# cropinghigh/sdrpp-dvbs-demodulator

Hardware: AMD Instinct MI355X
Metric: Msymbols/s demod+FEC, DVB-S2 8PSK 3/4 normal-frame @50 LDPC iters (higher is better)
Workload: dtype int8 (FEC) / f32 (demod); 1 GPU; DVB-S2 8PSK 3/4 normal FECFRAME (MODCOD 14), pilots off, 27.5 Msym/s-class streams at 2 sps, carrier offset 1e-3 rad/sample, clock error ~10 ppm, Es/N0 11 dB, 50 forced LDPC iterations, IQ in -> BBFRAMEs out; streams_per_gpu=4096, symbols_per_frame=21690, distinct_signal_blocks=64, parallelism=independent transponder streams sharded over GPUs, no data-path collective, fec_pipelined_across_steps=True, ranks_seen_by_backend=1, backend=none

## Files before the change

sdrpp-dvbs-demodulator_amd/csrc/bch_kernel.hip:

```cpp
#include <hip/hip_runtime.h>
#include <stdint.h>
#include "kernels.h"

namespace s2 {

struct GfDev {
    const uint16_t* __restrict__ LOG;
    const uint16_t* __restrict__ EXP;
    int N;
    __device__ __forceinline__ uint16_t imul(uint16_t a, uint16_t b) const {
        uint16_t tmp = (uint16_t)(a + b);
        return (N - (int)a <= (int)b) ? (uint16_t)(tmp - N) : tmp;
    }
    __device__ __forceinline__ uint16_t idiv(uint16_t a, uint16_t b) const {
        uint16_t tmp = (uint16_t)(a - b);
        return (a < b) ? (uint16_t)(tmp + N) : tmp;
    }
    __device__ __forceinline__ uint16_t vmul(uint16_t a, uint16_t b) const { return (!a || !b) ? (uint16_t)0 : EXP[imul(LOG[a], LOG[b])]; }
    __device__ __forceinline__ uint16_t vdiv(uint16_t a, uint16_t b) const { return !a ? (uint16_t)0 : EXP[idiv(LOG[a], LOG[b])]; }
    __device__ __forceinline__ uint16_t vmuli(uint16_t a, uint16_t idx) const { return !a ? (uint16_t)0 : EXP[imul(LOG[a], idx)]; }
};

__global__ __launch_bounds__(256) void bch_syndromes_kernel(BchDeviceCode C, const uint8_t* __restrict__ frames, int frame_stride,
                                                            int nbch, int nframes, uint16_t* __restrict__ syn_out, int32_t* __restrict__ todo,
                                                            int32_t* __restrict__ corrections) {
    __shared__ uint16_t tab[12 * 3 * 256];
    __shared__ uint16_t red[4][12];
    __shared__ uint16_t sfin[32];
    const int t = C.t;
    for (int i = threadIdx.x; i < t * 768; i += 256) tab[i] = C.d_syn_tab[i];
    __syncthreads();
    GfDev G{C.d_log, C.d_exp, C.N};
    const int nbytes = nbch / 8;
    const int chunk = (nbytes + 255) / 256;
    const int tid = threadIdx.x, lane = tid & 63, wave = tid >> 6;
    for (int f = blockIdx.x; f < nframes; f += gridDim.x) {
        const uint8_t* __restrict__ fr = frames + (size_t)f * frame_stride;
        int b0 = tid * chunk, b1 = min(b0 + chunk, nbytes);
        uint32_t P[12];
#pragma unroll
        for (int r = 0; r < 12; ++r) P[r] = 0;
        for (int b = b0; b < b1; ++b) {
            uint32_t byte = fr[b];
#pragma unroll
            for (int r = 0; r < 12; ++r)
                if (r < t) {
                    const uint16_t* T = tab + r * 768;
                    P[r] = (uint32_t)T[256 + (P[r] & 0xff)] ^ (uint32_t)T[512 + (P[r] >> 8)] ^ (uint32_t)T[byte];
                }
        }
        const long after = (b1 > b0) ? (long)nbch - 8L * b1 : 0;
#pragma unroll
        for (int r = 0; r < 12; ++r)
            if (r < t) {
                uint32_t v = P[r];
                if (v) {
                    int sh = (int)(((long)(2 * r + 1) * after) % C.N);
                    int e = (int)G.LOG[v] + sh;
                    if (e >= C.N) e -= C.N;
                    v = G.EXP[e];
                }
#pragma unroll
                for (int o = 32; o > 0; o >>= 1) v ^= __shfl_xor((int)v, o);
                if (lane == 0) red[wave][r] = (uint16_t)v;
            }
        __syncthreads();
        if (tid == 0) {
            for (int i = 0; i < 32; ++i) sfin[i] = 0;
            int nz = 0;
            for (int r = 0; r < t; ++r) { sfin[2 * r] = (uint16_t)(red[0][r] ^ red[1][r] ^ red[2][r] ^ red[3][r]); nz |= sfin[2 * r]; }
            if (nz)
                for (int k = 1; k <= t; ++k) sfin[2 * k - 1] = G.vmul(sfin[k - 1], sfin[k - 1]);
            sfin[31] = nz ? 1 : 0;
            if (nz) todo[2 + atomicAdd(&todo[0], 1)] = f;
            else if (corrections) corrections[f] = 0;
        }
        __syncthreads();
        if (tid < 32) syn_out[(size_t)f * 32 + tid] = sfin[tid];
        __syncthreads();
    }
}

__device__ __forceinline__ void xor_be_bit(uint8_t* buf, int pos) { buf[pos / 8] ^= (uint8_t)(1u << (7 - pos % 8)); }

constexpr int BCH_CT = 256;
constexpr int BCH_MAXDEG = 24;
__global__ __launch_bounds__(BCH_CT) void bch_correct_kernel(BchDeviceCode C, uint8_t* __restrict__ frames, int frame_stride, int nbch,
                                                             int kbch, int nframes, const uint16_t* __restrict__ syn_in, int32_t* __restrict__ todo,
                                                             int32_t* __restrict__ corrections) {
    __shared__ int s_item;
    __shared__ uint16_t s_loc[32];
    __shared__ uint16_t s_pos[32];
    __shared__ int s_deg, s_count, s_state;
    __shared__ uint16_t s_C[40], s_B[40], s_d;
    __shared__ uint16_t s_ev[32], s_mag[32];
    __shared__ int s_edeg;
    __shared__ uint16_t s_mul[BCH_MAXDEG][2][256];
    GfDev G{C.d_log, C.d_exp, C.N};
    const int NR = 2 * C.t;
    const int lane = threadIdx.x;
    const int ntodo = todo[0];
    while (true) {
        if (lane == 0) s_item = atomicAdd(&todo[1], 1);
        __syncthreads();
        const int item = s_item;
        __syncthreads();
        if (item >= ntodo) break;
        const int f = todo[2 + item];
        const uint16_t* __restrict__ syn = syn_in + (size_t)f * 32;
        if (lane <= NR) { s_C[lane] = lane == 0 ? 1 : 0; s_B[lane] = lane == 0 ? 1 : 0; }
        if (lane == 0) { s_state = 0; s_count = 0; s_deg = 0; }
        __syncthreads();
        int L = 0;
        for (int n = 0, m = 1; n < NR; ++n) {
            uint32_t prod = 0;
            if (lane >= 1 && lane <= L) prod = G.vmul(s_C[lane], syn[n - lane]);
            if (lane == 0) prod = syn[n];
#pragma unroll
            for (int o = 32; o > 0; o >>= 1) prod ^= (uint32_t)__shfl_xor((int)prod, o);
            if (lane == 0) s_d = (uint16_t)prod;
            __syncthreads();
            const uint16_t d = s_d;
            if (!d) {
                ++m;
            } else {
                uint16_t tnew = 0;
                if (lane <= NR) tnew = lane < m ? s_C[lane] : (uint16_t)(G.vmul(d, s_B[lane - m]) ^ s_C[lane]);
                const bool grow = 2 * L <= n;
                uint16_t bnew = 0;
                if (grow && lane <= NR) bnew = G.vdiv(s_C[lane], d);
                __syncthreads();
                if (lane <= NR) { s_C[lane] = tnew; if (grow) s_B[lane] = bnew; }
                if (grow) { L = n + 1 - L; m = 1; } else ++m;
            }
            __syncthreads();
        }
        if (lane == 0) {
            const uint16_t* Cc = s_C;
            int nonzero = 1;
            if (nonzero) {
                int deg = L;
                bool fail = false;
                while (!Cc[deg])
                    if (--deg < 0) { fail = true; break; }
                if (fail) {
                    s_state = -1;
                } else {
                    for (int i = 0; i <= NR; ++i) s_loc[i] = Cc[i];
                    s_deg = deg;
                    if (deg == 1) {
                        s_pos[0] = G.idiv(G.idiv(G.LOG[Cc[0]], G.LOG[Cc[1]]), 1);
                        s_count = 1; s_state = 2;
                    } else if (deg == 2) {
                        s_state = 2;
                        if (!Cc[1] || !Cc[0]) {
                            s_count = 0;
                        } else {
                            uint16_t a = Cc[2], b = Cc[1], c = Cc[0];
                            uint16_t ba = G.vdiv(b, a);
                            uint16_t Rr = C.d_imap[G.vdiv(G.vmul(a, c), G.vmul(b, b))];
                            if (!Rr) {
                                s_count = 0;
                            } else {
                                uint16_t v0 = G.vmul(ba, Rr);
                                s_pos[0] = G.idiv(G.LOG[v0], 1);
                                s_pos[1] = G.idiv(G.LOG[(uint16_t)(v0 ^ ba)], 1);
                                s_count = 2;
                            }
                        }
                    } else {
                        s_state = 1;
                    }
                }
            }
        }
        __syncthreads();
        if (s_state == 1) {
            const int deg = s_deg;
            for (int e = lane; e < deg * 512; e += BCH_CT) {
                const int j = e >> 9, h = (e >> 8) & 1, x = e & 255;
                const uint32_t v = h ? (uint32_t)x << 8 : (uint32_t)x;
                uint16_t r = 0;
                if (v && v <= (uint32_t)C.N) {
                    const int sh = (int)(((long)BCH_CT * (j + 1)) % C.N);
                    int lg2 = (int)G.LOG[v] + sh;
                    if (lg2 >= C.N) lg2 -= C.N;
                    r = G.EXP[lg2];
                }
                s_mul[j][h][x] = r;
            }
            uint32_t term[BCH_MAXDEG];
#pragma unroll
            for (int jj = 0; jj < BCH_MAXDEG; ++jj) {
                term[jj] = 0;
                if (jj < deg) {
                    const uint16_t c = s_loc[jj + 1];
                    if (c) {
                        const long e = (long)G.LOG[c] + (long)(jj + 1) * (long)(lane + 1);
                        term[jj] = G.EXP[(int)(e % C.N)];
                    }
                }
            }
            __syncthreads();
            const uint32_t c0 = s_loc[0];
            for (int i = lane; i < C.N; i += BCH_CT) {
                uint32_t sum = c0;
#pragma unroll
                for (int jj = 0; jj < BCH_MAXDEG; ++jj)
                    if (jj < deg) {
                        sum ^= term[jj];
                        term[jj] = (uint32_t)s_mul[jj][0][term[jj] & 255u] ^ (uint32_t)s_mul[jj][1][term[jj] >> 8];
                    }
                if (!sum) {
                    int slot = atomicAdd(&s_count, 1);
                    if (slot < 32) s_pos[slot] = (uint16_t)i;
                }
            }
            __syncthreads();
            if (lane == 0) s_state = 2;
        }
        __syncthreads();
        if (s_state == 2 && s_count >= s_deg && s_count <= 32 && s_count > 0) {
            const int count = s_count;
            const int etmp = count < NR - 1 ? count : NR - 1;
            if (lane <= etmp) {
                uint16_t e = G.vmul(syn[lane], s_loc[0]);
                for (int jj = 1; jj <= lane; ++jj) e ^= G.vmul(syn[lane - jj], s_loc[jj]);
                s_ev[lane] = e;
            }
            __syncthreads();
            if (lane == 0) {
                int edeg = -1;
                for (int i = 0; i <= etmp; ++i)
                    if (s_ev[i]) edeg = i;
                s_edeg = edeg;
            }
            __syncthreads();
            if (lane < count) {
                const int edeg = s_edeg;
                uint16_t root = G.imul(s_pos[lane], 1), tmp = root;
                uint16_t eval = s_ev[0];
                for (int jj = 1; jj <= edeg; ++jj) {
                    eval ^= G.vmuli(s_ev[jj], tmp);
                    tmp = G.imul(tmp, root);
                }
                uint16_t mag = 0;
                if (eval) {
                    uint16_t deriv = s_loc[1];
                    uint16_t root2 = G.imul(root, root), tmp2 = root2;
                    for (int jj = 3; jj <= count; jj += 2) {
                        deriv ^= G.vmuli(s_loc[jj], tmp2);
                        tmp2 = G.imul(tmp2, root2);
                    }
                    mag = G.EXP[G.idiv(G.LOG[eval], G.LOG[deriv])];
                }
                s_mag[lane] = mag;
            }
        }
        __syncthreads();
        if (lane == 0) {
            int result = 0;
            if (s_state == -1) {
                result = -1;
            } else if (s_state == 2) {
                const int deg = s_deg, count = s_count;
                if (count < deg || count > 32) {
                    result = -1;
                } else {
                    const uint16_t* magnitudes = s_mag;
                    const int short_by = C.K_full - kbch;
                    if (count <= 0) {
                        result = count;
                    } else {
                        bool bad = false;
                        for (int i = 0; i < count; ++i)
                            if ((int)s_pos[i] < short_by) bad = true;
                        if (!bad)
                            for (int i = 0; i < count; ++i)
                                if (1 < (int)magnitudes[i]) bad = true;
                        if (bad) {
                            result = -1;
                        } else {
                            uint8_t* fr = frames + (size_t)f * frame_stride;
                            for (int i = 0; i < count; ++i)
                                if (magnitudes[i]) { xor_be_bit(fr, (int)s_pos[i] - short_by); ++result; }
                        }
                    }
                }
            }
            if (corrections) corrections[f] = result;
        }
        __syncthreads();
    }
}

__global__ __launch_bounds__(256) void bb_descramble_kernel(const uint8_t* __restrict__ frames, int frame_stride,
                                                            const uint8_t* __restrict__ prbs, int out_bytes, int nframes,
                                                            uint8_t* __restrict__ out) {
    for (int f = blockIdx.y; f < nframes; f += gridDim.y)
        for (int b = blockIdx.x * 256 + threadIdx.x; b < out_bytes; b += gridDim.x * 256)
            out[(size_t)f * out_bytes + b] = frames[(size_t)f * frame_stride + b] ^ prbs[b];
}

hipError_t bch_syndromes_launch(const BchDeviceCode& C, const uint8_t* frames, int frame_stride, int nbch, int nframes,
                                uint16_t* syn, int32_t* todo, int32_t* corrections, hipStream_t stream) {
    hipError_t e = hipMemsetAsync(todo, 0, 2 * sizeof(int32_t), stream);
    if (e != hipSuccess) return e;
    int grid = nframes < 4096 ? nframes : 4096;
    hipLaunchKernelGGL(bch_syndromes_kernel, dim3(grid), dim3(256), 0, stream, C, frames, frame_stride, nbch, nframes, syn, todo, corrections);
    return hipGetLastError();
}
hipError_t bch_correct_launch(const BchDeviceCode& C, uint8_t* frames, int frame_stride, int nbch, int kbch, int nframes,
                              const uint16_t* syn, int32_t* todo, int32_t* corrections, hipStream_t stream) {
    int grid = nframes < 2048 ? nframes : 2048;
    hipLaunchKernelGGL(bch_correct_kernel, dim3(grid), dim3(BCH_CT), 0, stream, C, frames, frame_stride, nbch, kbch, nframes, syn, todo, corrections);
    return hipGetLastError();
}
hipError_t bb_descramble_launch(const uint8_t* frames, int frame_stride, const uint8_t* prbs, int out_bytes, int nframes,
                                uint8_t* out, hipStream_t stream) {
    int gx = (out_bytes + 255) / 256;
    if (gx > 32) gx = 32;
    int gy = nframes < 2048 ? nframes : 2048;
    hipLaunchKernelGGL(bb_descramble_kernel, dim3(gx, gy), dim3(256), 0, stream, frames, frame_stride, prbs, out_bytes, nframes, out);
    return hipGetLastError();
}

}
```

sdrpp-dvbs-demodulator_amd/csrc/capi.hip:

```cpp
#include "ctx.h"
#include <algorithm>
#include <climits>
#include <cstdlib>

using namespace s2;

namespace s2 {
std::atomic<long long> g_kernel_launches{0};
static thread_local std::string g_err;
std::string& last_error() { return g_err; }
int fail_hip(hipError_t e, const char* what) {
    g_err = std::string(what) + ": " + hipGetErrorString(e);
    return DVBS2GPU_ERR_HIP;
}
int dev_alloc(void** p, size_t bytes, bool zero, const char* what) {
    *p = nullptr;
    hipError_t e = hipMalloc(p, bytes);
    if (e == hipSuccess && zero) e = hipMemset(*p, 0, bytes);
    if (e == hipSuccess) return 0;
    dev_free(*p);
    *p = nullptr;
    return fail_hip(e, what);
}
void dev_free(void* p) { if (p) (void)hipFree(p); }
// ... 115 lines not shown
            if (!x || !y) return 0;
            int e = LOG[x] + LOG[y];
            if (e >= N) e -= N;
            return EXP[e];
        };
        for (int i = 2; i < N; i += 2) {
            uint16_t x = (uint16_t)i;
            uint16_t xxx = (uint16_t)(vmul(x, x) ^ x);
            if (xxx == (uint16_t)N) continue;
            IMAP[xxx] = x;
        }
        std::vector<uint16_t> tab((size_t)t * 768, 0);
        for (int r = 0; r < t; ++r) {
            int i = 2 * r + 1;
            uint16_t* T = &tab[(size_t)r * 768];
            for (int byte = 0; byte < 256; ++byte) {
                uint16_t v = 0;
                for (int b = 0; b < 8; ++b)
                    if ((byte >> (7 - b)) & 1) v ^= EXP[(int)(((long)i * (7 - b)) % N)];
                T[byte] = v;
            }
            uint16_t c = EXP[(int)(((long)i * 8) % N)];
            for (int x = 0; x < 256; ++x) {
                T[256 + x] = vmul((uint32_t)x, c);
                uint32_t hi = (uint32_t)x << 8;
                T[512 + x] = (hi < (uint32_t)Q) ? vmul(hi, c) : 0;
            }
        }
        BchCode D;
        D.m = m; D.t = t; D.N = N; D.K_full = N - m * t;
        int rc;
        if ((rc = upload(LOG, D.log, &D.d_log))) return rc;
        if ((rc = upload(EXP, D.exp, &D.d_exp))) return rc;
        if ((rc = upload(IMAP, D.imap, &D.d_imap))) return rc;
        if ((rc = upload(tab, D.syn_tab, &D.d_syn_tab))) return rc;
        it = ctx->bch.emplace(key, std::move(D)).first;
    }
    *out = &it->second;
    return 0;
}

// ... 3 lines not shown
    std::vector<uint8_t> seq(64800 / 8, 0);
    int sr = 0x4A80;
    for (int i = 0; i < 64800; i++) {
        int b = ((sr) ^ (sr >> 1)) & 1;
        seq[i / 8] |= (uint8_t)(b << (7 - (i % 8)));
        sr >>= 1;
        if (b) sr |= 0x4000;
    }
    return upload(seq, ctx->d_prbs);
}
}

namespace s2 {
static int ldpc_run(dvbs2gpu_ctx* ctx, const FecParams& f, const int8_t* d_llr, int nframes, int max_trials, int force,
                    uint8_t* d_hard, int hard_stride, int8_t* d_post, int32_t* d_trials, hipStream_t st, FecWs& W);
static int bch_run(dvbs2gpu_ctx* ctx, const FecParams& f, uint8_t* d_frames, int nframes, int32_t* d_corr, hipStream_t st, FecWs& W);

int fec_run(dvbs2gpu_ctx* ctx, const FecParams& f, const int8_t* d_llr, int nframes, int max_trials, int force, uint8_t* d_bbframes,
            int32_t* d_trials, int32_t* d_corr, hipStream_t st, FecWs* ws) {
    FecWs& W = ws ? *ws : ctx->fws;
    int rc;
    if ((rc = W.hard.ensure((size_t)nframes * (f.K / 8)))) return rc;
    uint8_t* hard = (uint8_t*)W.hard.p;
    {
        StageSpan sp(ctx->timers, ST_LDPC, st, nframes);
        if ((rc = ldpc_run(ctx, f, d_llr, nframes, max_trials, force, hard, f.K / 8, nullptr, d_trials, st, W))) return rc;
    }
    StageSpan sp(ctx->timers, ST_BCH, st, nframes);
    if ((rc = bch_run(ctx, f, hard, nframes, d_corr, st, W))) return rc;
    if ((rc = get_prbs(ctx))) return rc;
    HIP_TRY(bb_descramble_launch(hard, f.K / 8, ctx->d_prbs, f.kbch / 8, nframes, d_bbframes, st));
    return 0;
}
}

namespace s2 {
struct alignas(256) LdpcWorkCounter { unsigned int v[64]; };

enum class LdpcForm : int { lane = 0, wave = 1, split = 2 };
static LdpcForm ldpc_form(const dvbs2gpu_ctx* ctx, const LdpcDeviceCode& C) { return C.use_wave ? LdpcForm::wave : (C.use_split && ctx->ldpc_split) ? LdpcForm::split : LdpcForm::lane; }
struct LdpcGeometry { int grid, fpb; size_t rec_bytes; };
static LdpcGeometry ldpc_geometry(const dvbs2gpu_ctx* ctx, const LdpcDeviceCode& C, LdpcForm form, int nframes) {
    if (form == LdpcForm::wave) {
        const int per_cu = (int)((size_t)(160 * 1024 - LDPC_WAVE_LDS_RESERVE) / ldpc_wave_lds_bytes(C));
        return {std::min(ctx->num_cus * std::min(std::max(per_cu, 1), 16), nframes), 1, ldpc_wave_msg_bytes_per_frame(C)};
    }
    if (form == LdpcForm::split) return {std::min(ctx->num_cus * C.split_blocks_per_cu, nframes), 1, ldpc_split_msg_bytes_per_block(C)};
// ... 19 lines not shown
    }
    if (!d_hard) {
        if ((rc = W.hard.ensure((size_t)nframes * (f.K / 8)))) return rc;
        d_hard = (uint8_t*)W.hard.p; hard_stride = f.K / 8;
    }
    const LdpcJob J = {d_llr, nframes, max_trials, force, d_hard, hard_stride, d_post, d_trials, (uint32_t*)l_msg(W.msg.p), l_sgn(W.msg.p), l_counter(W.msg.p)->v,
                       G.grid, G.fpb, ctx->ldpc_split_fail_attempts, st};
    if (form == LdpcForm::wave) HIP_TRY(ldpc_wave_decode_launch(*C, J));
    else if (form == LdpcForm::lane) HIP_TRY(ldpc_decode_launch(*C, J));
    else if (nframes > 0) HIP_TRY(ldpc_split_decode_launch(*C, J));
    return 0;
}
}

namespace s2 {
static int bch_run(dvbs2gpu_ctx* ctx, const FecParams& f, uint8_t* d_frames, int nframes, int32_t* d_corr, hipStream_t st, FecWs& W) {
    BchDeviceCode* B;
    int rc = get_bch(ctx, f.bch_m, f.bch_t, &B);
    if (rc) return rc;
    ScratchLayout L;
    const auto l_syn = L.add<uint16_t>((size_t)nframes * 32); const auto l_todo = L.add<int32_t>((size_t)nframes + 2);
    if ((rc = W.syn.ensure(L.bytes()))) return rc;
    uint16_t* syn = l_syn(W.syn.p); int32_t* todo = l_todo(W.syn.p);
    HIP_TRY(bch_syndromes_launch(*B, d_frames, f.K / 8, f.K, nframes, syn, todo, d_corr, st));
    HIP_TRY(bch_correct_launch(*B, d_frames, f.K / 8, f.K, f.kbch, nframes, syn, todo, d_corr, st));
    return 0;
}
}

extern "C" {

const char* dvbs2gpu_version(void) { return "dvbs2gpu 0.1 (gfx950)"; }
int dvbs2gpu_preinit(void) {
    if (getenv("GPU_MAX_HW_QUEUES")) return 0;
    return setenv("GPU_MAX_HW_QUEUES", "12", 0) == 0 ? 1 : DVBS2GPU_ERR_ARG;
}
const char* dvbs2gpu_last_error(void) { return g_err.c_str(); }

int dvbs2gpu_device_count(void) {
    int n = 0;
// ... 259 lines not shown
    return rc ? rc : rc2;
}


int dvbs2gpu_bch_decode_batch(dvbs2gpu_ctx* ctx, int rate, int shortframes, uint8_t* d_frames, int nframes, int32_t* d_corrections,
                              void* stream) {
    if (!ctx || nframes < 0) return DVBS2GPU_ERR_ARG;
    FecParams f;
    if (!fec_params(rate, shortframes, &f)) { g_err = "unsupported code rate"; return DVBS2GPU_ERR_MODCOD; }
    if (nframes == 0) return 0;
    if (!d_frames) return DVBS2GPU_ERR_ARG;
    CallGuard guard(ctx);
    HIP_TRY(hipSetDevice(ctx->device));
    int rc = stage_enter(ctx, (hipStream_t)stream);
    if (rc) return rc;
    rc = bch_run(ctx, f, d_frames, nframes, d_corrections, (hipStream_t)stream, ctx->fws);
    int rc2 = ws_release(ctx, (hipStream_t)stream);
    return rc ? rc : rc2;
}

int dvbs2gpu_bb_descramble_batch(dvbs2gpu_ctx* ctx, int rate, int shortframes, const uint8_t* d_frames, int nframes, uint8_t* d_out,
                                 void* stream) {
    if (!ctx || nframes < 0) return DVBS2GPU_ERR_ARG;
    FecParams f;
    if (!fec_params(rate, shortframes, &f)) { g_err = "unsupported code rate"; return DVBS2GPU_ERR_MODCOD; }
    if (nframes == 0) return 0;
    if (!d_frames || !d_out) return DVBS2GPU_ERR_ARG;
    HIP_TRY(hipSetDevice(ctx->device));
    int rc = get_prbs(ctx);
    if (rc) return rc;
    HIP_TRY(bb_descramble_launch(d_frames, f.K / 8, ctx->d_prbs, f.kbch / 8, nframes, d_out, (hipStream_t)stream));
// ... 21 lines not shown
```

sdrpp-dvbs-demodulator_amd/csrc/kernels.h:

```cpp
#pragma once
#include <hip/hip_runtime.h>
#include <stdint.h>
#include "launch_count.h"

namespace s2 {

struct LdpcLayerDesc;

struct LdpcDeviceCode {
    int code_index = -1;
    int N = 0, K = 0, R = 0, q = 0, max_deg = 0, irregular = 0, rec_dwords = 0, edges = 0, pent_base = 0, synd_base = 0;
    LdpcLayerDesc* d_layers = nullptr;
    uint32_t* d_ents = nullptr;
    uint32_t* d_rows = nullptr;
    uint32_t* d_atab = nullptr;
    int blocks_per_cu = 1;
    int wave_lw = 0, wave_nsteps = 0, wave_nl_min = 0, wave_absent_base = 0;
    uint32_t* d_wave_lanec = nullptr;
    uint16_t* d_wave_steps = nullptr;
    uint32_t* d_wave_layer_end = nullptr;
    bool use_wave = false;
    struct LdpcSplitLayer* d_split_layers = nullptr;
    uint32_t* d_split_atab = nullptr;
    int split_npl = 0, split_rec_total = 0, split_blocks_per_cu = 1, split_tab_words = 0;
// ... 25 lines not shown
int ldpc_split_blocks_per_cu(int max_deg, int N);
size_t ldpc_split_msg_bytes_per_block(const LdpcDeviceCode& C);
hipError_t ldpc_split_decode_launch(const LdpcDeviceCode& C, const LdpcJob& J);
size_t ldpc_wave_msg_bytes_per_frame(const LdpcDeviceCode& C);
size_t ldpc_wave_lds_bytes(const LdpcDeviceCode& C);
hipError_t ldpc_wave_decode_launch(const LdpcDeviceCode& C, const LdpcJob& J);

struct BchDeviceCode {
    int m = 0, t = 0, N = 0;
    int K_full = 0;
    uint16_t* d_log = nullptr;
    uint16_t* d_exp = nullptr;
    uint16_t* d_imap = nullptr;
    uint16_t* d_syn_tab = nullptr;
};

hipError_t bch_syndromes_launch(const BchDeviceCode& C, const uint8_t* frames, int frame_stride, int nbch, int nframes,
                                uint16_t* syn , int32_t* todo, int32_t* corrections, hipStream_t stream);
hipError_t bch_correct_launch(const BchDeviceCode& C, uint8_t* frames, int frame_stride, int nbch, int kbch, int nframes,
                              const uint16_t* syn, int32_t* todo, int32_t* corrections, hipStream_t stream);
hipError_t bb_descramble_launch(const uint8_t* frames, int frame_stride, const uint8_t* prbs, int out_bytes, int nframes,
                                uint8_t* out, hipStream_t stream);

struct DvbsVitState {
    int state, rate, phase, shift, invalid;
    float ber;
    int dec_ss[10], dec_biased[10];
    int enc_state[5];
    int dep_first[2], dep_shift[2], dep_extra[2], dep_buf[2];
};
struct DvbsVitStats {
    float ber;
    int state, rate, phase, shift;
};
constexpr int DVBS_VIT_WS_BER_ENC = 2048 + 8192 + 64;
// ... 54 lines not shown
```

Baseline: 2849 Msymbols/s.

## Fuse BCH syndrome, correction and BB descrambling into one persistent tail kernel

Replaces the separate BCH syndrome kernel, BCH correction kernel and BB descramble kernel with a single templated persistent kernel that stages each frame in LDS, computes syndromes, corrects errors and descrambles to the output. The syndrome tables are rebuilt on the host as a minimal-polynomial remainder form, and the Chien search gets a two-positions-per-step variant for small degrees. The aim is to cut the extra launches, the global syndrome and todo buffers, and the repeated reads of frames from global memory. The cost is a much more complex kernel with heavy LDS use, which may limit occupancy.

Result: no change. 2862 Msymbols/s, median of 6 (+0.5%).

```diff
diff --git a/sdrpp-dvbs-demodulator_amd/csrc/bch_kernel.hip b/sdrpp-dvbs-demodulator_amd/csrc/bch_kernel.hip
--- a/sdrpp-dvbs-demodulator_amd/csrc/bch_kernel.hip
+++ b/sdrpp-dvbs-demodulator_amd/csrc/bch_kernel.hip
@@ -21,162 +21,151 @@
     __device__ __forceinline__ uint16_t vmuli(uint16_t a, uint16_t idx) const { return !a ? (uint16_t)0 : EXP[imul(LOG[a], idx)]; }
 };
 
-__global__ __launch_bounds__(256) void bch_syndromes_kernel(BchDeviceCode C, const uint8_t* __restrict__ frames, int frame_stride,
-                                                            int nbch, int nframes, uint16_t* __restrict__ syn_out, int32_t* __restrict__ todo,
-                                                            int32_t* __restrict__ corrections) {
-    __shared__ uint16_t tab[12 * 3 * 256];
-    __shared__ uint16_t red[4][12];
-    __shared__ uint16_t sfin[32];
-    const int t = C.t;
-    for (int i = threadIdx.x; i < t * 768; i += 256) tab[i] = C.d_syn_tab[i];
-    __syncthreads();
-    GfDev G{C.d_log, C.d_exp, C.N};
-    const int nbytes = nbch / 8;
-    const int chunk = (nbytes + 255) / 256;
-    const int tid = threadIdx.x, lane = tid & 63, wave = tid >> 6;
-    for (int f = blockIdx.x; f < nframes; f += gridDim.x) {
-        const uint8_t* __restrict__ fr = frames + (size_t)f * frame_stride;
-        int b0 = tid * chunk, b1 = min(b0 + chunk, nbytes);
-        uint32_t P[12];
-#pragma unroll
-        for (int r = 0; r < 12; ++r) P[r] = 0;
-        for (int b = b0; b < b1; ++b) {
-            uint32_t byte = fr[b];
-#pragma unroll
-            for (int r = 0; r < 12; ++r)
-                if (r < t) {
-                    const uint16_t* T = tab + r * 768;
-                    P[r] = (uint32_t)T[256 + (P[r] & 0xff)] ^ (uint32_t)T[512 + (P[r] >> 8)] ^ (uint32_t)T[byte];
-                }
-        }
-        const long after = (b1 > b0) ? (long)nbch - 8L * b1 : 0;
-#pragma unroll
-        for (int r = 0; r < 12; ++r)
-            if (r < t) {
-                uint32_t v = P[r];
-                if (v) {
-                    int sh = (int)(((long)(2 * r + 1) * after) % C.N);
-                    int e = (int)G.LOG[v] + sh;
-                    if (e >= C.N) e -= C.N;
-                    v = G.EXP[e];
-                }
-#pragma unroll
-                for (int o = 32; o > 0; o >>= 1) v ^= __shfl_xor((int)v, o);
-                if (lane == 0) red[wave][r] = (uint16_t)v;
-            }
-        __syncthreads();
-        if (tid == 0) {
-            for (int i = 0; i < 32; ++i) sfin[i] = 0;
-            int nz = 0;
-            for (int r = 0; r < t; ++r) { sfin[2 * r] = (uint16_t)(red[0][r] ^ red[1][r] ^ red[2][r] ^ red[3][r]); nz |= sfin[2 * r]; }
-            if (nz)
-                for (int k = 1; k <= t; ++k) sfin[2 * k - 1] = G.vmul(sfin[k - 1], sfin[k - 1]);
-            sfin[31] = nz ? 1 : 0;
-            if (nz) todo[2 + atomicAdd(&todo[0], 1)] = f;
-            else if (corrections) corrections[f] = 0;
-        }
-        __syncthreads();
-        if (tid < 32) syn_out[(size_t)f * 32 + tid] = sfin[tid];
-        __syncthreads();
-    }
-}
-
 __device__ __forceinline__ void xor_be_bit(uint8_t* buf, int pos) { buf[pos / 8] ^= (uint8_t)(1u << (7 - pos % 8)); }
 
 constexpr int BCH_CT = 256;
 constexpr int BCH_MAXDEG = 24;
-__global__ __launch_bounds__(BCH_CT) void bch_correct_kernel(BchDeviceCode C, uint8_t* __restrict__ frames, int frame_stride, int nbch,
-                                                             int kbch, int nframes, const uint16_t* __restrict__ syn_in, int32_t* __restrict__ todo,
-                                                             int32_t* __restrict__ corrections) {
-    __shared__ int s_item;
-    __shared__ uint16_t s_loc[32];
-    __shared__ uint16_t s_pos[32];
-    __shared__ int s_deg, s_count, s_state;
-    __shared__ uint16_t s_C[40], s_B[40], s_d;
-    __shared__ uint16_t s_ev[32], s_mag[32];
-    __shared__ int s_edeg;
-    __shared__ uint16_t s_mul[BCH_MAXDEG][2][256];
-    GfDev G{C.d_log, C.d_exp, C.N};
+constexpr int BCH_FRAME_LDS = BCH_MAX_FRAME_BYTES + 32;
+static_assert(BCH_MAX_FRAME_BYTES % 16 == 0, "the staged frame is addressed in 16-byte vectors");
+
+__device__ __forceinline__ uint32_t dword_at(const uint32_t* __restrict__ w, int byte_off) {
+    const int i = byte_off >> 2;
+    return __builtin_amdgcn_alignbyte(w[i + 1], w[i], (uint32_t)byte_off & 3u);
+}
+
+typedef unsigned short u16x2 __attribute__((ext_vector_type(2)));
+
+struct BchCorrLds {
+    uint16_t loc[32];
+    uint16_t pos[32];
+    uint16_t C[40], B[40], d;
+    uint16_t ev[32], mag[32];
+    int deg, count, state, edeg;
+};
+
+__device__ int bch_correct_frame(const BchDeviceCode& C, const GfDev& G, const uint16_t* syn, BchCorrLds& S, uint16_t* mul, int kbch,
+                                 uint8_t* __restrict__ fr, uint8_t* fr_lds) {
     const int NR = 2 * C.t;
     const int lane = threadIdx.x;
-    const int ntodo = todo[0];
-    while (true) {
-        if (lane == 0) s_item = atomicAdd(&todo[1], 1);
-        __syncthreads();
-        const int item = s_item;
-        __syncthreads();
-        if (item >= ntodo) break;
-        const int f = todo[2 + item];
-        const uint16_t* __restrict__ syn = syn_in + (size_t)f * 32;
-        if (lane <= NR) { s_C[lane] = lane == 0 ? 1 : 0; s_B[lane] = lane == 0 ? 1 : 0; }
-        if (lane == 0) { s_state = 0; s_count = 0; s_deg = 0; }
-        __syncthreads();
-        int L = 0;
-        for (int n = 0, m = 1; n < NR; ++n) {
-            uint32_t prod = 0;
-            if (lane >= 1 && lane <= L) prod = G.vmul(s_C[lane], syn[n - lane]);
-            if (lane == 0) prod = syn[n];
-#pragma unroll
-            for (int o = 32; o > 0; o >>= 1) prod ^= (uint32_t)__shfl_xor((int)prod, o);
-            if (lane == 0) s_d = (uint16_t)prod;
+    if (lane <= NR) { S.C[lane] = lane == 0 ? 1 : 0; S.B[lane] = lane == 0 ? 1 : 0; }
+    if (lane == 0) { S.state = 0; S.count = 0; S.deg = 0; }
+    __syncthreads();
+    int L = 0;
+    for (int n = 0, m = 1; n < NR; ++n) {
+        uint32_t prod = 0;
+        if (lane >= 1 && lane <= L) prod = G.vmul(S.C[lane], syn[n - lane]);
+        if (lane == 0) prod = syn[n];
+#pragma unroll
+        for (int o = 32; o > 0; o >>= 1) prod ^= (uint32_t)__shfl_xor((int)prod, o);
+        if (lane == 0) S.d = (uint16_t)prod;
+        __syncthreads();
+        const uint16_t d = S.d;
+        if (!d) {
+            ++m;
+        } else {
+            uint16_t tnew = 0;
+            if (lane <= NR) tnew = lane < m ? S.C[lane] : (uint16_t)(G.vmul(d, S.B[lane - m]) ^ S.C[lane]);
+            const bool grow = 2 * L <= n;
+            uint16_t bnew = 0;
+            if (grow && lane <= NR) bnew = G.vdiv(S.C[lane], d);
             __syncthreads();
-            const uint16_t d = s_d;
-            if (!d) {
-                ++m;
+            if (lane <= NR) { S.C[lane] = tnew; if (grow) S.B[lane] = bnew; }
+            if (grow) { L = n + 1 - L; m = 1; } else ++m;
+        }
+        __syncthreads();
+    }
+    if (lane == 0) {
+        const uint16_t* Cc = S.C;
+        int deg = L;
+        bool fail = false;
+        while (!Cc[deg])
+            if (--deg < 0) { fail = true; break; }
+        if (fail) {
+            S.state = -1;
+        } else {
+            for (int i = 0; i <= NR; ++i) S.loc[i] = Cc[i];
+            S.deg = deg;
+            if (deg == 1) {
+                S.pos[0] = G.idiv(G.idiv(G.LOG[Cc[0]], G.LOG[Cc[1]]), 1);
+                S.count = 1; S.state = 2;
+            } else if (deg == 2) {
+                S.state = 2;
+                if (!Cc[1] || !Cc[0]) {
+                    S.count = 0;
+                } else {
+                    uint16_t a = Cc[2], b = Cc[1], c = Cc[0];
+                    uint16_t ba = G.vdiv(b, a);
+                    uint16_t Rr = C.d_imap[G.vdiv(G.vmul(a, c), G.vmul(b, b))];
+                    if (!Rr) {
+                        S.count = 0;
+                    } else {
+                        uint16_t v0 = G.vmul(ba, Rr);
+                        S.pos[0] = G.idiv(G.LOG[v0], 1);
+                        S.pos[1] = G.idiv(G.LOG[(uint16_t)(v0 ^ ba)], 1);
+                        S.count = 2;
+                    }
+                }
             } else {
-                uint16_t tnew = 0;
-                if (lane <= NR) tnew = lane < m ? s_C[lane] : (uint16_t)(G.vmul(d, s_B[lane - m]) ^ s_C[lane]);
-                const bool grow = 2 * L <= n;
-                uint16_t bnew = 0;
-                if (grow && lane <= NR) bnew = G.vdiv(s_C[lane], d);
-                __syncthreads();
-                if (lane <= NR) { s_C[lane] = tnew; if (grow) s_B[lane] = bnew; }
-                if (grow) { L = n + 1 - L; m = 1; } else ++m;
+                S.state = 1;
+            }
+        }
+    }
+    __syncthreads();
+    if (S.state == 1) {
+        const int deg = S.deg;
+        const int i0 = C.K_full - kbch;
+        const uint32_t c0 = S.loc[0];
+        if (deg <= BCH_MAXDEG / 2) {
+            uint32_t* const mul32 = reinterpret_cast<uint32_t*>(mul);
+            for (int e = lane; e < deg * 512; e += BCH_CT) {
+                const int j = e >> 9, h = (e >> 8) & 1, x = e & 255;
+                const uint32_t v = h ? (uint32_t)x << 8 : (uint32_t)x;
+                uint32_t r = 0;
+                if (v && v <= (uint32_t)C.N) {
+                    const int sh = (int)(((long)BCH_CT * (j + 1)) % C.N);
+                    int l1 = (int)G.LOG[v] + sh;
+                    if (l1 >= C.N) l1 -= C.N;
+                    int l2 = l1 + sh;
+                    if (l2 >= C.N) l2 -= C.N;
+                    r = (uint32_t)G.EXP[l1] | ((uint32_t)G.EXP[l2] << 16);
+                }
+                mul32[e] = r;
+            }
+            uint32_t term[BCH_MAXDEG / 2];
+            uint32_t sum = c0;
+#pragma unroll
+            for (int jj = 0; jj < BCH_MAXDEG / 2; ++jj) {
+                term[jj] = 0;
+                if (jj < deg) {
+                    const uint16_t c = S.loc[jj + 1];
+                    if (c) {
+                        const long e = (long)G.LOG[c] + (long)(jj + 1) * (long)(i0 + lane + 1);
+                        term[jj] = G.EXP[(int)(e % C.N)];
+                    }
+                    sum ^= term[jj];
+                }
             }
             __syncthreads();
-        }
-        if (lane == 0) {
-            const uint16_t* Cc = s_C;
-            int nonzero = 1;
-            if (nonzero) {
-                int deg = L;
-                bool fail = false;
-                while (!Cc[deg])
-                    if (--deg < 0) { fail = true; break; }
-                if (fail) {
-                    s_state = -1;
-                } else {
-                    for (int i = 0; i <= NR; ++i) s_loc[i] = Cc[i];
-                    s_deg = deg;
-                    if (deg == 1) {
-                        s_pos[0] = G.idiv(G.idiv(G.LOG[Cc[0]], G.LOG[Cc[1]]), 1);
-                        s_count = 1; s_state = 2;
-                    } else if (deg == 2) {
-                        s_state = 2;
-                        if (!Cc[1] || !Cc[0]) {
-                            s_count = 0;
-                        } else {
-                            uint16_t a = Cc[2], b = Cc[1], c = Cc[0];
-                            uint16_t ba = G.vdiv(b, a);
-                            uint16_t Rr = C.d_imap[G.vdiv(G.vmul(a, c), G.vmul(b, b))];
-                            if (!Rr) {
-                                s_count = 0;
-                            } else {
-                                uint16_t v0 = G.vmul(ba, Rr);
-                                s_pos[0] = G.idiv(G.LOG[v0], 1);
-                                s_pos[1] = G.idiv(G.LOG[(uint16_t)(v0 ^ ba)], 1);
-                                s_count = 2;
-                            }
-                        }
-                    } else {
-                        s_state = 1;
-                    }
-                }
-            }
-        }
-        __syncthreads();
-        if (s_state == 1) {
-            const int deg = s_deg;
+            for (int i = i0 + lane; i < C.N; i += 2 * BCH_CT) {
+                uint32_t X = 0;
+#pragma unroll
+                for (int jj = 0; jj < BCH_MAXDEG / 2; ++jj)
+                    if (jj < deg) {
+                        const uint32_t two = mul32[jj * 512 + (term[jj] & 255u)] ^ mul32[jj * 512 + 256 + (term[jj] >> 8)];
+                        X ^= two;
+                        term[jj] = two >> 16;
+                    }
+                if (!sum) {
+                    int slot = atomicAdd(&S.count, 1);
+                    if (slot < 32) S.pos[slot] = (uint16_t)i;
+                }
+                if (((X & 0xffffu) ^ c0) == 0 && i + BCH_CT < C.N) {
+                    int slot = atomicAdd(&S.count, 1);
+                    if (slot < 32) S.pos[slot] = (uint16_t)(i + BCH_CT);
+                }
+                sum = c0 ^ (X >> 16);
+            }
+        } else {
             for (int e = lane; e < deg * 512; e += BCH_CT) {
                 const int j = e >> 9, h = (e >> 8) & 1, x = e & 255;
                 const uint32_t v = h ? (uint32_t)x << 8 : (uint32_t)x;
@@ -187,110 +176,245 @@
                     if (lg2 >= C.N) lg2 -= C.N;
                     r = G.EXP[lg2];
                 }
-                s_mul[j][h][x] = r;
+                mul[e] = r;
             }
             uint32_t term[BCH_MAXDEG];
 #pragma unroll
             for (int jj = 0; jj < BCH_MAXDEG; ++jj) {
                 term[jj] = 0;
                 if (jj < deg) {
-                    const uint16_t c = s_loc[jj + 1];
+                    const uint16_t c = S.loc[jj + 1];
                     if (c) {
-                        const long e = (long)G.LOG[c] + (long)(jj + 1) * (long)(lane + 1);
+                        const long e = (long)G.LOG[c] + (long)(jj + 1) * (long)(i0 + lane + 1);
                         term[jj] = G.EXP[(int)(e % C.N)];
                     }
                 }
             }
             __syncthreads();
-            const uint32_t c0 = s_loc[0];
-            for (int i = lane; i < C.N; i += BCH_CT) {
+            for (int i = i0 + lane; i < C.N; i += BCH_CT) {
                 uint32_t sum = c0;
 #pragma unroll
                 for (int jj = 0; jj < BCH_MAXDEG; ++jj)
                     if (jj < deg) {
                         sum ^= term[jj];
-                        term[jj] = (uint32_t)s_mul[jj][0][term[jj] & 255u] ^ (uint32_t)s_mul[jj][1][term[jj] >> 8];
+                        term[jj] = (uint32_t)mul[jj * 512 + (term[jj] & 255u)] ^ (uint32_t)mul[jj * 512 + 256 + (term[jj] >> 8)];
                     }
                 if (!sum) {
-                    int slot = atomicAdd(&s_count, 1);
-                    if (slot < 32) s_pos[slot] = (uint16_t)i;
-                }
-            }
+                    int slot = atomicAdd(&S.count, 1);
+                    if (slot < 32) S.pos[slot] = (uint16_t)i;
+                }
+            }
+        }
+        __syncthreads();
+        if (lane == 0) S.state = 2;
+    }
+    __syncthreads();
+    if (S.state == 2 && S.count >= S.deg && S.count <= 32 && S.count > 0) {
+        const int count = S.count;
+        const int etmp = count < NR - 1 ? count : NR - 1;
+        if (lane <= etmp) {
+            uint16_t e = G.vmul(syn[lane], S.loc[0]);
+            for (int jj = 1; jj <= lane; ++jj) e ^= G.vmul(syn[lane - jj], S.loc[jj]);
+            S.ev[lane] = e;
+        }
+        __syncthreads();
+        if (lane == 0) {
+            int edeg = -1;
+            for (int i = 0; i <= etmp; ++i)
+                if (S.ev[i]) edeg = i;
+            S.edeg = edeg;
+        }
+        __syncthreads();
+        if (lane < count) {
+            const int edeg = S.edeg;
+            uint16_t root = G.imul(S.pos[lane], 1), tmp = root;
+            uint16_t eval = S.ev[0];
+            for (int jj = 1; jj <= edeg; ++jj) {
+                eval ^= G.vmuli(S.ev[jj], tmp);
+                tmp = G.imul(tmp, root);
+            }
+            uint16_t mag = 0;
+            if (eval) {
+                uint16_t deriv = S.loc[1];
+                uint16_t root2 = G.imul(root, root), tmp2 = root2;
+                for (int jj = 3; jj <= count; jj += 2) {
+                    deriv ^= G.vmuli(S.loc[jj], tmp2);
+                    tmp2 = G.imul(tmp2, root2);
+                }
+                mag = G.EXP[G.idiv(G.LOG[eval], G.LOG[deriv])];
+            }
+            S.mag[lane] = mag;
+        }
+    }
+    __syncthreads();
+    int result = 0;
+    if (lane == 0) {
+        if (S.state == -1) {
+            result = -1;
+        } else if (S.state == 2) {
+            const int deg = S.deg, count = S.count;
+            if (count < deg || count > 32) {
+                result = -1;
+            } else {
+                const uint16_t* magnitudes = S.mag;
+                const int short_by = C.K_full - kbch;
+                if (count <= 0) {
+                    result = count;
+                } else {
+                    bool bad = false;
+                    for (int i = 0; i < count; ++i)
+                        if ((int)S.pos[i] < short_by) bad = true;
+                    if (!bad)
+                        for (int i = 0; i < count; ++i)
+                            if (1 < (int)magnitudes[i]) bad = true;
+                    if (bad) {
+                        result = -1;
+                    } else {
+                        for (int i = 0; i < count; ++i)
+                            if (magnitudes[i]) { xor_be_bit(fr, (int)S.pos[i] - short_by); xor_be_bit(fr_lds, (int)S.pos[i] - short_by); ++result; }
+                    }
+                }
+            }
+        }
+    }
+    __syncthreads();
+    return result;
+}
+
+template <int T>
+__global__ __launch_bounds__(BCH_CT, 4) void bch_tail_kernel(
+BchDeviceCode C, uint8_t* __restrict__ frames, int frame_stride, int nbch, int kbch, int nframes,
+                                                          int32_t* __restrict__ corrections, const uint32_t* __restrict__ prbs, uint8_t* __restrict__ out,
+                                                          int out_bytes, unsigned int* __restrict__ ctr) {
+    __shared__ uint32_t s_tab32[BCH_MAXDEG * 256];
+    __shared__ uint4 s_frame4[BCH_FRAME_LDS / 16];
+    __shared__ uint32_t s_red[4][T / 2];
+    __shared__ uint16_t s_syn[32];
+    __shared__ BchCorrLds s_corr;
+    __shared__ int s_next;
+    static_assert(T % 2 == 0 && T * 768 <= BCH_MAXDEG * 512, "syndrome tables fit the Chien tables' LDS");
+    uint16_t* const s_tab = reinterpret_cast<uint16_t*>(s_tab32);
+    uint8_t* const s_frame = reinterpret_cast<uint8_t*>(s_frame4);
+    const uint32_t* const s_framew = reinterpret_cast<const uint32_t*>(s_frame4);
+    const GfDev G{C.d_log, C.d_exp, C.N};
+    const int tid = threadIdx.x, lane = tid & 63, wave = tid >> 6;
+    const int nbytes = nbch / 8;
+    const int chunk = ((nbytes + 255) / 256 + 3) & ~3;
+    const int hs = C.m - 8;
+    const uint32_t rmask2 = (((1u << C.m) - 1u) & ~0xffu) * 0x10001u;
+    const int b0 = min(tid * chunk, nbytes), b1 = min(b0 + chunk, nbytes);
+    const int sh1 = (int)(((long)nbch - 8L * b1) % C.N), sh2 = 2 * sh1 >= C.N ? 2 * sh1 - C.N : 2 * sh1;
+    bool tables = false;
+    int f = blockIdx.x;
+    while (f < nframes) {
+        if (tid == 0) s_next = (int)(gridDim.x + atomicAdd(&ctr[0], 1u));
+        if (!tables) {
+            for (int i = tid; i < T * 768; i += BCH_CT) s_tab[i] = C.d_syn_tab[i];
+            tables = true;
+        }
+        uint8_t* __restrict__ fr = frames + (size_t)f * frame_stride;
+        const int off = (int)((uintptr_t)fr & 15u);
+        {
+            const int head = min((16 - off) & 15, nbytes), nvec = (nbytes - head) >> 4;
+            if (tid < head) s_frame[off + tid] = fr[tid];
+            const uint4* __restrict__ src = reinterpret_cast<const uint4*>(fr + head);
+            uint4* dst = s_frame4 + ((off + head) >> 4);
+            for (int v = tid; v < nvec; v += BCH_CT) dst[v] = src[v];
+            const int done = head + 16 * nvec;
+            if (tid < nbytes - done) s_frame[off + done + tid] = fr[done + tid];
+        }
+        __syncthreads();
+        uint32_t PP[T / 2];
+#pragma unroll
+        for (int r = 0; r < T / 2; ++r) PP[r] = 0;
+        auto step = [&](uint32_t byte) {
+            const uint32_t b2 = byte | (byte << 16);
+#pragma unroll
+            for (int r = 0; r < T / 2; ++r) {
+                const u16x2 tv = {s_tab[(2 * r) * 768 + ((PP[r] >> hs) & 0xffu)], s_tab[(2 * r + 1) * 768 + (PP[r] >> (16 + hs))]};
+                PP[r] = ((PP[r] << 8) & rmask2) ^ __builtin_bit_cast(uint32_t, tv) ^ b2;
+            }
+        };
+        {
+            int b = b0, wi = (off + b0) >> 2;
+            const uint32_t sh = (uint32_t)(off + b0) & 3u;
+            uint32_t cur = s_framew[wi];
+            for (; b + 4 <= b1; b += 4) {
+                const uint32_t nxt = s_framew[++wi];
+                const uint32_t w = __builtin_amdgcn_alignbyte(nxt, cur, sh);
+                cur = nxt;
+                step(w & 0xffu); step((w >> 8) & 0xffu); step((w >> 16) & 0xffu); step(w >> 24);
+            }
+            for (; b < b1; ++b) step(s_frame[off + b]);
+        }
+        uint32_t P[T];
+#pragma unroll
+        for (int r = 0; r < T / 2; ++r) { P[2 * r] = PP[r] & 0xffffu; P[2 * r + 1] = PP[r] >> 16; }
+        int sh = sh1;
+#pragma unroll
+        for (int r = 0; r < T; ++r) {
+            uint32_t v = (uint32_t)s_tab[r * 768 + 256 + (P[r] & 0xffu)] ^ (uint32_t)s_tab[r * 768 + 512 + (P[r] >> 8)];
+            if (v) {
+                int e = (int)G.LOG[v] + sh;
+                if (e >= C.N) e -= C.N;
+                v = G.EXP[e];
+            }
+            P[r] = v;
+            sh += sh2;
+            if (sh >= C.N) sh -= C.N;
+        }
+#pragma unroll
+        for (int r = 0; r < T / 2; ++r) {
+            uint32_t v = P[2 * r] | (P[2 * r + 1] << 16);
+#pragma unroll
+            for (int o = 32; o > 0; o >>= 1) v ^= (uint32_t)__shfl_xor((int)v, o);
+            if (lane == 0) s_red[wave][r] = v;
+        }
+        __syncthreads();
+        uint32_t mine = 0;
+        if (tid < T) {
+            const uint32_t v = s_red[0][tid >> 1] ^ s_red[1][tid >> 1] ^ s_red[2][tid >> 1] ^ s_red[3][tid >> 1];
+            mine = (tid & 1) ? v >> 16 : v & 0xffffu;
+            s_syn[2 * tid] = (uint16_t)mine;
+        }
+        const int nz = __syncthreads_or((int)mine);
+        const int next = s_next;
+        if (nz) {
+            if (tid == 0)
+                for (int k = 1; k <= T; ++k) s_syn[2 * k - 1] = G.vmul(s_syn[k - 1], s_syn[k - 1]);
             __syncthreads();
-            if (lane == 0) s_state = 2;
-        }
-        __syncthreads();
-        if (s_state == 2 && s_count >= s_deg && s_count <= 32 && s_count > 0) {
-            const int count = s_count;
-            const int etmp = count < NR - 1 ? count : NR - 1;
-            if (lane <= etmp) {
-                uint16_t e = G.vmul(syn[lane], s_loc[0]);
-                for (int jj = 1; jj <= lane; ++jj) e ^= G.vmul(syn[lane - jj], s_loc[jj]);
-                s_ev[lane] = e;
-            }
-            __syncthreads();
-            if (lane == 0) {
-                int edeg = -1;
-                for (int i = 0; i <= etmp; ++i)
-                    if (s_ev[i]) edeg = i;
-                s_edeg = edeg;
-            }
-            __syncthreads();
-            if (lane < count) {
-                const int edeg = s_edeg;
-                uint16_t root = G.imul(s_pos[lane], 1), tmp = root;
-                uint16_t eval = s_ev[0];
-                for (int jj = 1; jj <= edeg; ++jj) {
-                    eval ^= G.vmuli(s_ev[jj], tmp);
-                    tmp = G.imul(tmp, root);
-                }
-                uint16_t mag = 0;
-                if (eval) {
-                    uint16_t deriv = s_loc[1];
-                    uint16_t root2 = G.imul(root, root), tmp2 = root2;
-                    for (int jj = 3; jj <= count; jj += 2) {
-                        deriv ^= G.vmuli(s_loc[jj], tmp2);
-                        tmp2 = G.imul(tmp2, root2);
-                    }
-                    mag = G.EXP[G.idiv(G.LOG[eval], G.LOG[deriv])];
-                }
-                s_mag[lane] = mag;
-            }
-        }
-        __syncthreads();
-        if (lane == 0) {
-            int result = 0;
-            if (s_state == -1) {
-                result = -1;
-            } else if (s_state == 2) {
-                const int deg = s_deg, count = s_count;
-                if (count < deg || count > 32) {
-                    result = -1;
-                } else {
-                    const uint16_t* magnitudes = s_mag;
-                    const int short_by = C.K_full - kbch;
-                    if (count <= 0) {
-                        result = count;
-                    } else {
-                        bool bad = false;
-                        for (int i = 0; i < count; ++i)
-                            if ((int)s_pos[i] < short_by) bad = true;
-                        if (!bad)
-                            for (int i = 0; i < count; ++i)
-                                if (1 < (int)magnitudes[i]) bad = true;
-                        if (bad) {
-                            result = -1;
-                        } else {
-                            uint8_t* fr = frames + (size_t)f * frame_stride;
-                            for (int i = 0; i < count; ++i)
-                                if (magnitudes[i]) { xor_be_bit(fr, (int)s_pos[i] - short_by); ++result; }
-                        }
-                    }
-                }
-            }
-            if (corrections) corrections[f] = result;
-        }
-        __syncthreads();
+            const int result = bch_correct_frame(C, G, s_syn, s_corr, s_tab, kbch, fr, s_frame + off);
+            if (tid == 0 && corrections) corrections[f] = result;
+            tables = false;
+        } else if (tid == 0 && corrections) {
+            corrections[f] = 0;
+        }
+        if (out) {
+            uint8_t* __restrict__ o = out + (size_t)f * out_bytes;
+            const uint8_t* __restrict__ prbs8 = reinterpret_cast<const uint8_t*>(prbs);
+            const int head = min((int)((16u - ((uintptr_t)o & 15u)) & 15u), out_bytes), nvec = (out_bytes - head) >> 4;
+            if (tid < head) o[tid] = s_frame[off + tid] ^ prbs8[tid];
+            for (int v = tid; v < nvec; v += BCH_CT) {
+                const int b = head + 16 * v;
+                uint4 x;
+                x.x = dword_at(s_framew, off + b) ^ dword_at(prbs, b);
+                x.y = dword_at(s_framew, off + b + 4) ^ dword_at(prbs, b + 4);
+                x.z = dword_at(s_framew, off + b + 8) ^ dword_at(prbs, b + 8);
+                x.w = dword_at(s_framew, off + b + 12) ^ dword_at(prbs, b + 12);
+                *reinterpret_cast<uint4*>(o + b) = x;
+            }
+            const int done = head + 16 * nvec;
+            if (tid < out_bytes - done) o[done + tid] = s_frame[off + done + tid] ^ prbs8[done + tid];
+        }
+        __syncthreads();
+        f = next;
+    }
+    if (tid == 0) {
+        __threadfence();
+        if (atomicAdd(&ctr[1], 1u) == gridDim.x - 1) {
+            atomicExch(&ctr[0], 0u);
+            atomicExch(&ctr[1], 0u);
+        }
     }
 }
 
@@ -302,19 +426,32 @@
             out[(size_t)f * out_bytes + b] = frames[(size_t)f * frame_stride + b] ^ prbs[b];
 }
 
-hipError_t bch_syndromes_launch(const BchDeviceCode& C, const uint8_t* frames, int frame_stride, int nbch, int nframes,
-                                uint16_t* syn, int32_t* todo, int32_t* corrections, hipStream_t stream) {
-    hipError_t e = hipMemsetAsync(todo, 0, 2 * sizeof(int32_t), stream);
-    if (e != hipSuccess) return e;
-    int grid = nframes < 4096 ? nframes : 4096;
-    hipLaunchKernelGGL(bch_syndromes_kernel, dim3(grid), dim3(256), 0, stream, C, frames, frame_stride, nbch, nframes, syn, todo, corrections);
+template <int T>
+static hipError_t bch_tail_launch_t(const BchDeviceCode& C, uint8_t* frames, int frame_stride, int nbch, int kbch, int nframes, int32_t* corrections,
+                                    const uint8_t* prbs, uint8_t* out, int out_bytes, unsigned int* ctr, int num_cus, hipStream_t stream) {
+    static int per_cu = 0;
+    if (!per_cu) {
+        int nb = 0;
+        if (hipOccupancyMaxActiveBlocksPerMultiprocessor(&nb, bch_tail_kernel<T>, BCH_CT, 0) != hipSuccess || nb < 1) nb = 1;
+        per_cu = nb;
+    }
+    const long cap = (long)num_cus * per_cu;
+    const int grid = (int)(nframes < cap ? nframes : cap);
+    hipLaunchKernelGGL(bch_tail_kernel<T>, dim3(grid), dim3(BCH_CT), 0, stream, C, frames, frame_stride, nbch, kbch, nframes, corrections,
+                       reinterpret_cast<const uint32_t*>(prbs), out, out_bytes, ctr);
     return hipGetLastError();
 }
-hipError_t bch_correct_launch(const BchDeviceCode& C, uint8_t* frames, int frame_stride, int nbch, int kbch, int nframes,
-                              const uint16_t* syn, int32_t* todo, int32_t* corrections, hipStream_t stream) {
-    int grid = nframes < 2048 ? nframes : 2048;
-    hipLaunchKernelGGL(bch_correct_kernel, dim3(grid), dim3(BCH_CT), 0, stream, C, frames, frame_stride, nbch, kbch, nframes, syn, todo, corrections);
-    return hipGetLastError();
+
+hipError_t bch_tail_launch(const BchDeviceCode& C, uint8_t* frames, int frame_stride, int nbch, int kbch, int nframes, int32_t* corrections,
+                           const uint8_t* prbs, uint8_t* out, int out_bytes, unsigned int* ctr, int num_cus, hipStream_t stream) {
+    if (nframes <= 0) return hipSuccess;
+    if (nbch / 8 > BCH_MAX_FRAME_BYTES || (out && (!prbs || out_bytes > nbch / 8 || ((uintptr_t)prbs & 3u)))) return hipErrorInvalidValue;
+    switch (C.t) {
+        case 8:  return bch_tail_launch_t<8>(C, frames, frame_stride, nbch, kbch, nframes, corrections, prbs, out, out_bytes, ctr, num_cus, stream);
+        case 10: return bch_tail_launch_t<10>(C, frames, frame_stride, nbch, kbch, nframes, corrections, prbs, out, out_bytes, ctr, num_cus, stream);
+        case 12: return bch_tail_launch_t<12>(C, frames, frame_stride, nbch, kbch, nframes, corrections, prbs, out, out_bytes, ctr, num_cus, stream);
+        default: return hipErrorInvalidValue;
+    }
 }
 hipError_t bb_descramble_launch(const uint8_t* frames, int frame_stride, const uint8_t* prbs, int out_bytes, int nframes,
                                 uint8_t* out, hipStream_t stream) {
diff --git a/sdrpp-dvbs-demodulator_amd/csrc/capi.hip b/sdrpp-dvbs-demodulator_amd/csrc/capi.hip
--- a/sdrpp-dvbs-demodulator_amd/csrc/capi.hip
+++ b/sdrpp-dvbs-demodulator_amd/csrc/capi.hip
@@ -153,17 +153,34 @@
         for (int r = 0; r < t; ++r) {
             int i = 2 * r + 1;
             uint16_t* T = &tab[(size_t)r * 768];
-            for (int byte = 0; byte < 256; ++byte) {
-                uint16_t v = 0;
-                for (int b = 0; b < 8; ++b)
-                    if ((byte >> (7 - b)) & 1) v ^= EXP[(int)(((long)i * (7 - b)) % N)];
-                T[byte] = v;
+            std::vector<uint16_t> mp(m + 1, 0);
+            mp[0] = 1;
+            long conj = i;
+            for (int k = 0; k < m; ++k) {
+                const uint16_t root = EXP[(int)(conj % N)];
+                for (int d = k + 1; d > 0; --d) mp[d] = (uint16_t)(mp[d - 1] ^ vmul(mp[d], root));
+                mp[0] = vmul(mp[0], root);
+                conj = (conj * 2) % N;
             }
-            uint16_t c = EXP[(int)(((long)i * 8) % N)];
+            uint32_t low = 0;
+            for (int d = 0; d <= m; ++d) {
+                if (mp[d] > 1 || (d == m && mp[d] != 1)) { g_err = "BCH tables: the conjugates of alpha^i do not give a binary polynomial of degree m"; return DVBS2GPU_ERR_ARG; }
+                if (d < m && mp[d]) low |= 1u << d;
+            }
+            for (int h = 0; h < 256; ++h) {
+                uint32_t v = (uint32_t)h << (m - 8);
+                for (int s = 0; s < 8; ++s) v = (v & (1u << (m - 1))) ? (((v << 1) ^ low) & (uint32_t)(Q - 1)) : (v << 1);
+                T[h] = (uint16_t)v;
+            }
             for (int x = 0; x < 256; ++x) {
-                T[256 + x] = vmul((uint32_t)x, c);
-                uint32_t hi = (uint32_t)x << 8;
-                T[512 + x] = (hi < (uint32_t)Q) ? vmul(hi, c) : 0;
+                uint16_t lo = 0, hi = 0;
+                for (int k = 0; k < 8; ++k)
+                    if ((x >> k) & 1) {
+                        lo ^= EXP[(int)(((long)i * k) % N)];
+                        if (8 + k < m) hi ^= EXP[(int)(((long)i * (8 + k)) % N)];
+                    }
+                T[256 + x] = lo;
+                T[512 + x] = hi;
             }
         }
         BchCode D;
@@ -197,7 +214,7 @@
 namespace s2 {
 static int ldpc_run(dvbs2gpu_ctx* ctx, const FecParams& f, const int8_t* d_llr, int nframes, int max_trials, int force,
                     uint8_t* d_hard, int hard_stride, int8_t* d_post, int32_t* d_trials, hipStream_t st, FecWs& W);
-static int bch_run(dvbs2gpu_ctx* ctx, const FecParams& f, uint8_t* d_frames, int nframes, int32_t* d_corr, hipStream_t st, FecWs& W);
+static int bch_run(dvbs2gpu_ctx* ctx, const FecParams& f, uint8_t* d_frames, int nframes, int32_t* d_corr, uint8_t* d_out, hipStream_t st, FecWs& W);
 
 int fec_run(dvbs2gpu_ctx* ctx, const FecParams& f, const int8_t* d_llr, int nframes, int max_trials, int force, uint8_t* d_bbframes,
             int32_t* d_trials, int32_t* d_corr, hipStream_t st, FecWs* ws) {
@@ -210,10 +227,7 @@
         if ((rc = ldpc_run(ctx, f, d_llr, nframes, max_trials, force, hard, f.K / 8, nullptr, d_trials, st, W))) return rc;
     }
     StageSpan sp(ctx->timers, ST_BCH, st, nframes);
-    if ((rc = bch_run(ctx, f, hard, nframes, d_corr, st, W))) return rc;
-    if ((rc = get_prbs(ctx))) return rc;
-    HIP_TRY(bb_descramble_launch(hard, f.K / 8, ctx->d_prbs, f.kbch / 8, nframes, d_bbframes, st));
-    return 0;
+    return bch_run(ctx, f, hard, nframes, d_corr, d_bbframes, st, W);
 }
 }
 
@@ -263,16 +277,16 @@
 }
 
 namespace s2 {
-static int bch_run(dvbs2gpu_ctx* ctx, const FecParams& f, uint8_t* d_frames, int nframes, int32_t* d_corr, hipStream_t st, FecWs& W) {
+static int bch_run(dvbs2gpu_ctx* ctx, const FecParams& f, uint8_t* d_frames, int nframes, int32_t* d_corr, uint8_t* d_out, hipStream_t st, FecWs& W) {
     BchDeviceCode* B;
     int rc = get_bch(ctx, f.bch_m, f.bch_t, &B);
     if (rc) return rc;
-    ScratchLayout L;
-    const auto l_syn = L.add<uint16_t>((size_t)nframes * 32); const auto l_todo = L.add<int32_t>((size_t)nframes + 2);
-    if ((rc = W.syn.ensure(L.bytes()))) return rc;
-    uint16_t* syn = l_syn(W.syn.p); int32_t* todo = l_todo(W.syn.p);
-    HIP_TRY(bch_syndromes_launch(*B, d_frames, f.K / 8, f.K, nframes, syn, todo, d_corr, st));
-    HIP_TRY(bch_correct_launch(*B, d_frames, f.K / 8, f.K, f.kbch, nframes, syn, todo, d_corr, st));
+    if (d_out && (rc = get_prbs(ctx))) return rc;
+    if (!W.syn.p) {
+        if ((rc = W.syn.ensure(64 * sizeof(unsigned int)))) return rc;
+        HIP_TRY(hipMemsetAsync(W.syn.p, 0, 64 * sizeof(unsigned int), st));
+    }
+    HIP_TRY(bch_tail_launch(*B, d_frames, f.K / 8, f.K, f.kbch, nframes, d_corr, ctx->d_prbs, d_out, f.kbch / 8, (unsigned int*)W.syn.p, ctx->num_cus, st));
     return 0;
 }
 }
@@ -562,7 +576,7 @@
     HIP_TRY(hipSetDevice(ctx->device));
     int rc = stage_enter(ctx, (hipStream_t)stream);
     if (rc) return rc;
-    rc = bch_run(ctx, f, d_frames, nframes, d_corrections, (hipStream_t)stream, ctx->fws);
+    rc = bch_run(ctx, f, d_frames, nframes, d_corrections, nullptr, (hipStream_t)stream, ctx->fws);
     int rc2 = ws_release(ctx, (hipStream_t)stream);
     return rc ? rc : rc2;
 }
diff --git a/sdrpp-dvbs-demodulator_amd/csrc/kernels.h b/sdrpp-dvbs-demodulator_amd/csrc/kernels.h
--- a/sdrpp-dvbs-demodulator_amd/csrc/kernels.h
+++ b/sdrpp-dvbs-demodulator_amd/csrc/kernels.h
@@ -63,11 +63,10 @@
     uint16_t* d_imap = nullptr;
     uint16_t* d_syn_tab = nullptr;
 };
+constexpr int BCH_MAX_FRAME_BYTES = 7296;
 
-hipError_t bch_syndromes_launch(const BchDeviceCode& C, const uint8_t* frames, int frame_stride, int nbch, int nframes,
-                                uint16_t* syn , int32_t* todo, int32_t* corrections, hipStream_t stream);
-hipError_t bch_correct_launch(const BchDeviceCode& C, uint8_t* frames, int frame_stride, int nbch, int kbch, int nframes,
-                              const uint16_t* syn, int32_t* todo, int32_t* corrections, hipStream_t stream);
+hipError_t bch_tail_launch(const BchDeviceCode& C, uint8_t* frames, int frame_stride, int nbch, int kbch, int nframes, int32_t* corrections,
+                           const uint8_t* prbs, uint8_t* out, int out_bytes, unsigned int* ctr, int num_cus, hipStream_t stream);
 hipError_t bb_descramble_launch(const uint8_t* frames, int frame_stride, const uint8_t* prbs, int out_bytes, int nframes,
                                 uint8_t* out, hipStream_t stream);
 
```
